# BGU-CS-VIL/DPMMSubClusters.jl

Hardware: AMD Instinct MI355X
Metric: Gibbs iterations/sec, N=10M D=64 NIW (higher is better)
Workload: dtype f32

## Files before the change

### dpmmsubclusters.jl_amd/csrc/dpmm_api.cpp

```cpp
#include "../../include/dpmm_hip.h"
#include "../../include/dpmm_hip_master.h"
#include "../../include/dpmm_hip_debug.h"
#include "../../include/dpmm_hip_tensor.h"
#include "../../include/dpmm_hip_csc.h"
#include "../../include/dpmm_hip_score.h"

#include <hip/hip_runtime.h>
#include <dlfcn.h>

#include <algorithm>
#include <atomic>
#include <condition_variable>
#include <mutex>
#include <thread>
#include <chrono>
#include <cmath>
#include <cstdio>
#include <cstring>
#include <cstdlib>
#include <ctime>
#include <string>
#include <unordered_map>
#include <vector>

// ... 1830 lines not shown
    }
    if (armed && wd_disarm(c)) {
        c->err = "collective timed out: a peer rank is gone or stuck (communicator aborted after DPMM_OPT_COMM_TIMEOUT_MS)";
        return DPMM_ECOMM;
    }
    if (c->comm_aborted.load(std::memory_order_relaxed) && rc == DPMM_OK && master_records_marked(sm, nrec)) return fail(c, DPMM_ECOMM, "communicator aborted");
    return rc;
}

int dpmm_debug_set_prelaunch_hook(void (*fn)(void *), void *arg) {
    dpmm::g_prelaunch_arg = arg;
    dpmm::g_prelaunch = fn;
    return DPMM_OK;
}

int dpmm_debug_counters(dpmm_ctx *c, int64_t *out, int n) {
    if (!c || !out || n < 1) return DPMM_EINVAL;
    for (int i = 0; i < n; ++i) out[i] = 0;
    out[0] = c->dbg_early_wait;
    return DPMM_OK;
}

int dpmm_step_master_device(dpmm_ctx *c, uint32_t reset_epoch, const int32_t *slots, uint32_t draw_epoch, const uint8_t **bad, const double **small) {
    if (!c || !slots || !bad || !small) return DPMM_EINVAL;
    if (!c->master) return fail(c, DPMM_ESTATE, "dpmm_niw_master_setup first");
    const int K = c->K;
    if (K < 1) return fail(c, DPMM_ESTATE, "no clusters");
    HIPCHK(c, hipSetDevice(c->device));
    int top = 0;
    for (int k = 0; k < K; ++k) {
        if (slots[k] < 0 || slots[k] >= DPMM_MAX_CLUSTERS) return fail(c, DPMM_EINVAL, "slot out of range");
        top = std::max(top, slots[k] + 1);
    }
    if (int rc = noise_flush(c)) return rc;
    if (int rc = master_capacity(c, top, draw_epoch ? K : 0)) return rc;
    if (int rc = spec_join(c)) return rc;
    c->spec_valid = false;
    const size_t out_bytes = sizeof(double) * 2 * (size_t)K * (size_t)c->packed_stride;
    if (int rc = ensure_out(c, DPMM_MAX_CLUSTERS + 64)) return rc;
    const size_t jobs_bytes = (sizeof(int32_t) * 2 * (size_t)K + 63) & ~(size_t)63;
    if (int rc = master_pinned(c, jobs_bytes + sizeof(double) * 3 * DPMM_MASTER_NSCALARS * (size_t)K)) return rc;
    std::vector<int32_t> jobs(2 * (size_t)K);
    for (int k = 0; k < K; ++k) { jobs[2 * k] = k; jobs[2 * k + 1] = slots[k]; }
    if (int rc = device_list(c, c->d_jobs, c->jobs_shadow, jobs.data(), jobs.size())) return rc;
    if (draw_epoch) if (int rc = device_list(c, c->d_dslots, c->dslots_shadow, slots, (size_t)K)) return rc;
    for (int32_t sl : c->apairs_req) if (sl >= top) { c->apairs_req.clear(); break; }
    const int napairs = (int)(c->apairs_req.size() / 2);
    c->apairs_valid = false;
    bool fuse_pairs = true;
    if (napairs > 0) {
        if ((size_t)napairs > c->apairs_cap) {
            HIPCHK(c, sync_stream(c, c->stream));
            HIPCHK(c, hipStreamSynchronize(c->stream2));
            size_t cap = 64;
            while (cap < (size_t)napairs) cap *= 2;
            hipFree(c->d_apairs); c->d_apairs = nullptr;
            if (c->h_apairs) hipHostFree(c->h_apairs);
            c->h_apairs = nullptr; c->apairs_cap = 0; c->apairs_shadow.clear();
            HIPCHK(c, hipMalloc(&c->d_apairs, sizeof(int32_t) * 2 * cap));
            HIPCHK(c, hipHostMalloc((void **)&c->h_apairs, sizeof(double) * DPMM_MASTER_NSCALARS * cap, hipHostMallocDefault));
            c->apairs_cap = cap;
        }
        if (c->ma.DP > 128 && (size_t)napairs > c->pair_cap) {
            HIPCHK(c, sync_stream(c, c->stream));
            HIPCHK(c, hipStreamSynchronize(c->stream2));
            hipFree(c->d_pairs); c->d_pairs = nullptr; c->pair_cap = 0;
            size_t cap = 64;
            while (cap < (size_t)napairs) cap *= 2;
            HIPCHK(c, hipMalloc(&c->d_pairs, sizeof(double) * cap * (size_t)c->ma.DP * (size_t)c->ma.DP));
            c->pair_cap = cap;
        }
        if (niw_master_can_fuse_pairs(c->ma)) {
            std::vector<int32_t> inv((size_t)top, -1), kp(c->apairs_req.size());
            for (int k = 0; k < K; ++k) inv[slots[k]] = k;
            for (size_t i = 0; i < kp.size(); ++i) {
                kp[i] = inv[c->apairs_req[i]];
                if (kp[i] < 0) { fuse_pairs = false; break; }
            }
            if (fuse_pairs) {
                if (c->opt_chain & 4) {
                    if (!(c->apairs_shadow.size() == kp.size() && memcmp(c->apairs_shadow.data(), kp.data(), sizeof(int32_t) * kp.size()) == 0) || !c->apairs_pinned_cur) {
                        c->apairs_shadow.assign(kp.begin(), kp.end());
                        c->apairs_pin_flip ^= 1;
                        int32_t *&buf = c->h_apairs_list[c->apairs_pin_flip];
                        size_t &cap = c->h_apairs_list_cap[c->apairs_pin_flip];
                        if (kp.size() > cap) {
                            if (buf) HIPCHK(c, hipHostFree(buf));
                            buf = nullptr; cap = 0;
                            size_t nc = 2048;
                            while (nc < kp.size()) nc *= 2;
                            HIPCHK(c, hipHostMalloc((void **)&buf, sizeof(int32_t) * nc, hipHostMallocDefault));
                            cap = nc;
                        }
                        memcpy(buf, kp.data(), sizeof(int32_t) * kp.size());
                        c->apairs_pinned_cur = buf;
                    }
                } else {
                    if (c->apairs_pinned_cur) { c->apairs_shadow.clear(); c->apairs_pinned_cur = nullptr; }
                    if (int rc = device_list(c, c->d_apairs, c->apairs_shadow, kp.data(), kp.size())) return rc;
                }
            }
        } else fuse_pairs = false;
        if (!fuse_pairs) {
            if (c->apairs_pinned_cur) { c->apairs_shadow.clear(); c->apairs_pinned_cur = nullptr; }
            if (int rc = device_list(c, c->d_apairs, c->apairs_shadow, c->apairs_req.data(), c->apairs_req.size(), c->stream2)) return rc;
        }
    } else fuse_pairs = false;
    double *sm = reinterpret_cast<double *>(c->h_master + jobs_bytes);
    master_mark_records(sm, 3 * (int64_t)K);
    const bool poll = c->opt_master_poll != 0;
    bool flags_sent = false;
    if (int rc = run_stats(c, nullptr, 0, true, reset_epoch, reinterpret_cast<uint8_t *>(c->h_out), &flags_sent)) return rc;
    if (!flags_sent) HIPCHK(c, launch_copy_bytes(c->h_out, reinterpret_cast<const uint8_t *>(c->d_out) + out_bytes, (size_t)K + 1, c->stream));
    const bool noise_in_post = draw_epoch != 0 && (c->opt_chain & 16) != 0 && niw_master_can_fuse_pairs(c->ma);
    bool normals_by_post = false;
    if (noise_in_post) {
        if (int rc = noise_join(c)) return rc;
        c->noise_valid = false;
    }
    if ((napairs > 0 && fuse_pairs) || noise_in_post) {
        const int nfp = fuse_pairs ? napairs : 0;
        if (poll && nfp > 0) master_mark_records(c->h_apairs, nfp);
        HIPCHK(c, launch_niw_master_posterior_pairs(c->ma, c->d_jobs, K, c->d_out, sm, ((c->opt_chain & 4) && c->apairs_pinned_cur) ? c->apairs_pinned_cur : c->d_apairs, nfp, c->h_apairs, c->stream,
                                                    noise_in_post ? 3 * K : 0, draw_epoch, noise_in_post ? c->d_Y[c->draw_cur ^ 1] : nullptr));
        normals_by_post = noise_in_post;
    } else HIPCHK(c, launch_niw_master_posterior(c->ma, c->d_jobs, K, c->d_out, sm, c->stream));
    if (napairs > 0 && fuse_pairs) {
        c->apairs_index.clear();
        for (int p = 0; p < napairs; ++p) c->apairs_index[((uint32_t)c->apairs_req[2 * p] << 16) | (uint32_t)c->apairs_req[2 * p + 1]] = p;
        c->apairs_dirty.assign((size_t)c->master_slots, 0);
        c->apairs_inflight = false; c->apairs_valid = true;
        c->apairs_req.clear();
    }
    const bool fused_pairs_launched = napairs > 0 && fuse_pairs;
    const bool need_event = !poll || (napairs > 0 && !fuse_pairs);
    if (need_event) HIPCHK(c, hipEventRecord(c->ev_master, c->stream));
    if (napairs > 0 && !fuse_pairs) {
        HIPCHK(c, hipStreamWaitEvent(c->stream2, c->ev_master, 0));
        HIPCHK(c, launch_niw_master_pairs(c->ma, c->d_apairs, napairs, c->d_pairs, c->h_apairs, c->stream2));
        HIPCHK(c, hipEventRecord(c->ev_pairs, c->stream2));
        c->apairs_index.clear();
        for (int p = 0; p < napairs; ++p) c->apairs_index[((uint32_t)c->apairs_req[2 * p] << 16) | (uint32_t)c->apairs_req[2 * p + 1]] = p;
        c->apairs_dirty.assign((size_t)c->master_slots, 0);
        c->apairs_inflight = true; c->apairs_valid = true;
        c->apairs_req.clear();
    }
    if (draw_epoch) {
        const int32_t *hs = c->d_dslots;
        const bool have_normals = normals_by_post || noise_ready(c, draw_epoch, K, c->draw_cur ^ 1);
        if (int rc = noise_join(c)) return rc;
        NiwMasterArgs ma = c->ma;
        ma.mu_draw = c->d_mu_draw[c->draw_cur ^ 1];
        HIPCHK(c, launch_niw_master_draw(ma, hs, K, draw_epoch, c->d_Y[c->draw_cur ^ 1], c->d_ld_sigma[c->draw_cur ^ 1], nullptr, nullptr,
                                         nullptr, nullptr, nullptr, nullptr, c->NB, nullptr, 1 | (have_normals ? 4 : 0), c->stream));
        c->noise_valid = false;
        c->spec_inflight = false; c->spec_valid = true; c->spec_epoch = draw_epoch;
        c->spec_slots.assign(slots, slots + K);
    }
    if (int rc = flush_undo(c)) return rc;
    if (poll) { if (int rc = wait_master_records(c, sm, 3 * (int64_t)K, c->h_apairs, fused_pairs_launched ? napairs : 0)) return rc; }
    else HIPCHK(c, sync_event(c, c->ev_master));
    if (master_marks_left(sm, K)) {
        ++c->dbg_early_wait;
        const auto t0 = std::chrono::steady_clock::now();
        while (master_marks_left(sm, K)) {
            if (std::chrono::steady_clock::now() - t0 > std::chrono::seconds(5)) return fail(c, DPMM_EHIP, "posterior records missing 5 s after the event wait returned");
            HIPCHK(c, sync_stream(c, c->stream));
        }
    }
    c->handover_inflight = false;
    *bad = reinterpret_cast<const uint8_t *>(c->h_out);
    *small = sm;
    return DPMM_OK;
}

int dpmm_suffstats_device(dpmm_ctx *c, const int64_t *idx, int n_idx) {
    if (!c) return DPMM_EINVAL;
    if (!c->master) return fail(c, DPMM_ESTATE, "dpmm_niw_master_setup first");
    return run_stats(c, idx, n_idx);
}

int dpmm_niw_master_posterior(dpmm_ctx *c, const int64_t *clusters, const int32_t *slots, int n, const double **small) {
    if (!c || !slots || !small || n < 0) return DPMM_EINVAL;
    if (!c->master) return fail(c, DPMM_ESTATE, "dpmm_niw_master_setup first");
    if (n == 0) { *small = nullptr; return DPMM_OK; }
    HIPCHK(c, hipSetDevice(c->device));
    int top = 0;
    for (int i = 0; i < n; ++i) {
        const int64_t k = clusters ? clusters[i] : i + 1;
        if (k < 1 || k > c->K) return fail(c, DPMM_EINVAL, "cluster index out of range");
        if (slots[i] < 0 || slots[i] >= DPMM_MAX_CLUSTERS) return fail(c, DPMM_EINVAL, "slot out of range");
        top = std::max(top, slots[i] + 1);
    }
    if (int rc = master_capacity(c, top, 0)) return rc;
    if (int rc = spec_join(c)) return rc;
    c->spec_valid = false;
    for (int i = 0; i < n; ++i) if ((size_t)slots[i] < c->apairs_dirty.size()) c->apairs_dirty[slots[i]] = 1;
    const size_t jobs_bytes = (sizeof(int32_t) * 2 * (size_t)n + 63) & ~(size_t)63;
    if (int rc = master_pinned(c, jobs_bytes + sizeof(double) * 3 * DPMM_MASTER_NSCALARS * (size_t)n)) return rc;
    HIPCHK(c, sync_stream(c, c->stream));
    std::vector<int32_t> jobs(2 * (size_t)n);
    for (int i = 0; i < n; ++i) { jobs[2 * i] = (int32_t)((clusters ? clusters[i] : i + 1) - 1); jobs[2 * i + 1] = slots[i]; }
    if (int rc = device_list(c, c->d_jobs, c->jobs_shadow, jobs.data(), jobs.size())) return rc;
    double *sm = reinterpret_cast<double *>(c->h_master + jobs_bytes);
    HIPCHK(c, launch_niw_master_posterior(c->ma, c->d_jobs, n, c->d_out, sm, c->stream));
    HIPCHK(c, sync_stream(c, c->stream));
    *small = sm;
    return DPMM_OK;
}

int dpmm_niw_master_draw(dpmm_ctx *c, uint32_t epoch, int K, const int32_t *slot_of_cluster, const float *lr, const float *w) {
    if (!c || !slot_of_cluster || !lr || !w) return DPMM_EINVAL;
    if (!c->master) return fail(c, DPMM_ESTATE, "dpmm_niw_master_setup first");
    if (int rc = check_K(c, K)) return rc;
    HIPCHK(c, hipSetDevice(c->device));
    for (int k = 0; k < K; ++k)
        if (slot_of_cluster[k] < 0 || slot_of_cluster[k] >= c->master_slots) return fail(c, DPMM_EINVAL, "slot without a posterior on the device");
    if (int rc = noise_flush(c)) return rc;
    if (int rc = ensure_capacity(c, K)) return rc;
    if (int rc = master_capacity(c, 0, K)) return rc;
    if (c->handover_inflight) HIPCHK(c, sync_stream(c, c->stream));
    c->handover_inflight = true;
    float *hlr = reinterpret_cast<float *>(c->h_draw), *hw = hlr + 2 * K;
    memcpy(hlr, lr, sizeof(float) * 2 * K);
    memcpy(hw, w, sizeof(float) * K);
    c->have_tail = c->opt_tail && c->D >= 4 && c->D % 4 == 0 && K > 1;
    const bool ahead = c->spec_valid && c->spec_epoch == epoch && (int)c->spec_slots.size() == K &&
                       memcmp(c->spec_slots.data(), slot_of_cluster, sizeof(int32_t) * K) == 0;
    if (int rc = spec_join(c)) return rc;
    c->spec_valid = false;
    if (int rc = noise_join(c)) return rc;
    if (!ahead) if (int rc = device_list(c, c->d_dslots, c->dslots_shadow, slot_of_cluster, (size_t)K)) return rc;
    const int32_t *hs = c->d_dslots;
    c->draw_cur ^= 1;
    NiwMasterArgs ma = c->ma;
    ma.mu_draw = c->d_mu_draw[c->draw_cur];
    const bool normals = !ahead && noise_ready(c, epoch, K, c->draw_cur);
    c->predictive = false;
    const bool roles = (c->opt_chain & 2) != 0, b3_in_pack = roles && want_b3_images(c), pb_in_pack = b3_in_pack && want_pair_ball(c, K);
    HIPCHK(c, launch_niw_master_draw(ma, hs, K, epoch, c->d_Y[c->draw_cur], c->d_ld_sigma[c->draw_cur], hlr, hw, c->d_Rp, c->d_mup, c->d_cst,
                                     c->have_tail ? c->d_tail : nullptr, c->NB, c->d_work, (ahead ? 2 : (normals ? 7 : 3)) | (roles ? 8 : 0) | (b3_in_pack ? 16 : 0) | (pb_in_pack ? 32 : 0), c->stream));
    if (int rc = direction_tables(c, K, b3_in_pack, pb_in_pack)) return rc;
    c->noise_pending = c->opt_noise_ahead < 0 ? (c->D >= 128 || c->n < 4000000) : c->opt_noise_ahead != 0; c->noise_pend_epoch = epoch + 1; c->noise_pend_nmat = 3 * std::min(K + 4, c->master_K);
    if ((c->opt_chain & 16) && niw_master_can_fuse_pairs(c->ma)) c->noise_pending = false;
    c->work_zeroed = true;
    c->have_screen_prep = false;
    c->K = K;
    c->have_params = true;
    c->predictive = false;
    c->draws_on_device = true;
    return DPMM_OK;
}

int dpmm_niw_master_pairs_ahead(dpmm_ctx *c, const int32_t *slots_i, const int32_t *slots_j, int n) {
    if (!c || n < 0 || (n > 0 && (!slots_i || !slots_j))) return DPMM_EINVAL;
    if (!c->master) return fail(c, DPMM_ESTATE, "dpmm_niw_master_setup first");
    c->apairs_req.clear();
    for (int i = 0; i < n; ++i) {
        if (slots_i[i] < 0 || slots_i[i] >= DPMM_MAX_CLUSTERS || slots_j[i] < 0 || slots_j[i] >= DPMM_MAX_CLUSTERS) { c->apairs_req.clear(); return fail(c, DPMM_EINVAL, "slot out of range"); }
        c->apairs_req.push_back(slots_i[i]); c->apairs_req.push_back(slots_j[i]);
    }
    return DPMM_OK;
}

int dpmm_niw_master_pairs(dpmm_ctx *c, const int32_t *slots_i, const int32_t *slots_j, int n, const double **small) {
    if (!c || !slots_i || !slots_j || !small || n < 0) return DPMM_EINVAL;
    if (!c->master) return fail(c, DPMM_ESTATE, "dpmm_niw_master_setup first");
    if (n == 0) { *small = nullptr; return DPMM_OK; }
    HIPCHK(c, hipSetDevice(c->device));
    for (int i = 0; i < n; ++i)
        if (slots_i[i] < 0 || slots_i[i] >= c->master_slots || slots_j[i] < 0 || slots_j[i] >= c->master_slots) return fail(c, DPMM_EINVAL, "slot out of range");
    const size_t DP = (size_t)c->ma.DP;
    if (c->apairs_valid) {
        bool all = true;
        std::vector<int> rec((size_t)n);
        for (int i = 0; i < n && all; ++i) {
            const auto it = c->apairs_index.find(((uint32_t)slots_i[i] << 16) | (uint32_t)slots_j[i]);
            all = it != c->apairs_index.end() && !c->apairs_dirty[slots_i[i]] && !c->apairs_dirty[slots_j[i]];
            if (all) rec[i] = it->second;
        }
        if (all) {
            if (int rc = master_pinned(c, sizeof(double) * DPMM_MASTER_NSCALARS * (size_t)n)) return rc;
            HIPCHK(c, hipEventSynchronize(c->ev_pairs));
            double *sm = reinterpret_cast<double *>(c->h_master);
            for (int i = 0; i < n; ++i) memcpy(sm + (size_t)i * DPMM_MASTER_NSCALARS, c->h_apairs + (size_t)rec[i] * DPMM_MASTER_NSCALARS, sizeof(double) * DPMM_MASTER_NSCALARS);
            *small = sm;
            return DPMM_OK;
        }
    }
    if (int rc = spec_join(c)) return rc;
    if ((size_t)n > c->pair_cap) {
        HIPCHK(c, sync_stream(c, c->stream));
        HIPCHK(c, hipStreamSynchronize(c->stream2));
        hipFree(c->d_pairs); c->d_pairs = nullptr; c->pair_cap = 0;
        size_t cap = 64;
        while (cap < (size_t)n) cap *= 2;
        HIPCHK(c, hipMalloc(&c->d_pairs, sizeof(double) * cap * DP * DP));
        c->pair_cap = cap;
    }
    const size_t idx_bytes = (sizeof(int32_t) * 2 * (size_t)n + 63) & ~(size_t)63;
    if (int rc = master_pinned(c, idx_bytes + sizeof(double) * DPMM_MASTER_NSCALARS * (size_t)n)) return rc;
    HIPCHK(c, sync_stream(c, c->stream));
    int32_t *pr = reinterpret_cast<int32_t *>(c->h_master);
    for (int i = 0; i < n; ++i) { pr[2 * i] = slots_i[i]; pr[2 * i + 1] = slots_j[i]; }
    double *sm = reinterpret_cast<double *>(c->h_master + idx_bytes);
    HIPCHK(c, launch_niw_master_pairs(c->ma, pr, n, c->d_pairs, sm, c->stream));
    HIPCHK(c, sync_stream(c, c->stream));
    *small = sm;
    return DPMM_OK;
}

int dpmm_niw_master_put_rows(dpmm_ctx *c, const double *rows, int K) {
    if (!c || !rows) return DPMM_EINVAL;
    if (!c->master) return fail(c, DPMM_ESTATE, "dpmm_niw_master_setup first");
    if (int rc = check_K(c, K)) return rc;
    HIPCHK(c, hipSetDevice(c->device));
    if (int rc = ensure_capacity(c, K)) return rc;
    HIPCHK(c, sync_stream(c, c->stream));
    HIPCHK(c, hipMemcpy(c->d_out, rows, sizeof(double) * 2 * (size_t)K * (size_t)c->packed_stride, hipMemcpyHostToDevice));
    c->apairs_valid = false;
    if (K != c->K) c->have_params = false;
    c->K = K;
    return DPMM_OK;
}

int dpmm_niw_master_rows(dpmm_ctx *c, const int32_t *slots, int n, double *out) {
    if (!c || !slots || !out || n < 0) return DPMM_EINVAL;
    if (!c->master) return fail(c, DPMM_ESTATE, "dpmm_niw_master_setup first");
    if (n == 0) return DPMM_OK;
    HIPCHK(c, hipSetDevice(c->device));
    const size_t stride = (size_t)c->packed_stride, bytes = sizeof(double) * 2 * (size_t)n * stride;
    for (int i = 0; i < n; ++i)
        if (slots[i] < 0 || slots[i] >= c->master_slots) return fail(c, DPMM_EINVAL, "slot out of range");
    if (int rc = ensure_out(c, bytes)) return rc;
    if (int rc = ensure_pinned(c, sizeof(int32_t) * (size_t)n + 64)) return rc;
    HIPCHK(c, sync_stream(c, c->stream));
    memcpy(c->h_pin, slots, sizeof(int32_t) * (size_t)n);
    HIPCHK(c, launch_niw_rows_gather(c->ma.rows_store, reinterpret_cast<const int32_t *>(c->h_pin), n, (int64_t)stride,
                                     reinterpret_cast<double *>(c->h_out), c->stream));
    HIPCHK(c, sync_stream(c, c->stream));
    memcpy(out, c->h_out, bytes);
    return DPMM_OK;
}

int dpmm_niw_master_draws(dpmm_ctx *c, int K, float *mu, float *R, float *logdet) {
    if (!c || !mu || !R || !logdet) return DPMM_EINVAL;
    if (!c->master || !c->draws_on_device || K != c->K) return fail(c, DPMM_ESTATE, "no device draws for this K");
    HIPCHK(c, hipSetDevice(c->device));
    HIPCHK(c, sync_stream(c, c->stream));
    const size_t D = (size_t)c->D, DP = (size_t)c->ma.DP;
    std::vector<double> Y(3 * (size_t)K * DP * DP);
    std::vector<float> m(3 * (size_t)K * DP);
    HIPCHK(c, hipMemcpy(Y.data(), c->d_Y[c->draw_cur], sizeof(double) * Y.size(), hipMemcpyDeviceToHost));
    HIPCHK(c, hipMemcpy(m.data(), c->d_mu_draw[c->draw_cur], sizeof(float) * m.size(), hipMemcpyDeviceToHost));
    HIPCHK(c, hipMemcpy(logdet, c->d_ld_sigma[c->draw_cur], sizeof(float) * 3 * (size_t)K, hipMemcpyDeviceToHost));
    for (size_t j = 0; j < 3 * (size_t)K; ++j) {
        for (size_t d = 0; d < D; ++d) mu[j * D + d] = m[j * DP + d];
        for (size_t r = 0; r < D; ++r)
            for (size_t cc = 0; cc < D; ++cc) R[(j * D + r) * D + cc] = cc >= r ? (float)Y[(j * DP + cc) * DP + r] : 0.f;
    }
    return DPMM_OK;
}

int dpmm_mult_master_setup(dpmm_ctx *c, const float *alpha, const float *alpha_outlier) {
    if (!c || !alpha) return DPMM_EINVAL;
    if (c->prior != DPMM_PRIOR_MULT) return fail(c, DPMM_EINVAL, "dpmm_mult_master_setup: the context is not Multinomial");
    if (c->D > DPMM_MULT_MASTER_MAXD) return fail(c, DPMM_ELIMIT, "D exceeds the device Dirichlet draw's limit");
    HIPCHK(c, hipSetDevice(c->device));
    HIPCHK(c, sync_stream(c, c->stream));
    if (!c->d_malpha) HIPCHK(c, hipMalloc(&c->d_malpha, sizeof(float) * 2 * (size_t)c->ldx));
    HIPCHK(c, hipMemsetAsync(c->d_malpha, 0, sizeof(float) * 2 * (size_t)c->ldx, c->stream));
    HIPCHK(c, sync_stream(c, c->stream));
    HIPCHK(c, hipMemcpy(c->d_malpha, alpha, sizeof(float) * (size_t)c->D, hipMemcpyHostToDevice));
    if (alpha_outlier) HIPCHK(c, hipMemcpy(c->d_malpha + c->ldx, alpha_outlier, sizeof(float) * (size_t)c->D, hipMemcpyHostToDevice));
    c->mult_has_alpha1 = alpha_outlier != nullptr;
    for (int p = 0; p < 2; ++p) {
        const float *al = p ? alpha_outlier : alpha;
        double sa = 0.0, sl = 0.0;
        if (al) for (int d = 0; d < c->D; ++d) { sa += (double)al[d]; sl += lgamma((double)al[d]); }
        c->mult_prior_c[2 * p] = sa; c->mult_prior_c[2 * p + 1] = sl;
    }
    if (!c->d_mpairs) HIPCHK(c, hipMalloc(&c->d_mpairs, sizeof(int32_t) * 2 * DPMM_MULT_MASTER_MAXPAIRS));
    if (!c->h_marg) HIPCHK(c, hipHostMalloc((void **)&c->h_marg, sizeof(double) * (6 * DPMM_MAX_CLUSTERS + DPMM_MULT_MASTER_MAXPAIRS), hipHostMallocDefault));
    c->marg_valid = false; c->marg_req = false; c->mpairs_shadow.clear();
    if (!c->h_draw) HIPCHK(c, hipHostMalloc((void **)&c->h_draw, sizeof(float) * 3 * DPMM_MAX_CLUSTERS, hipHostMallocDefault));
    c->mult_master = true;
    return DPMM_OK;
}

int dpmm_mult_master_put_rows(dpmm_ctx *c, const double *rows, int K) {
    if (!c || !rows) return DPMM_EINVAL;
    if (!c->mult_master) return fail(c, DPMM_ESTATE, "dpmm_mult_master_setup first");
    if (int rc = check_K(c, K)) return rc;
    HIPCHK(c, hipSetDevice(c->device));
// ... 1063 lines not shown
```

### dpmmsubclusters.jl_amd/csrc/niw_master.hip

```cpp
#include <algorithm>
#include "dpmm_device.h"
#include "dpmm_kernels.h"
#include "niw_b3.h"

namespace dpmm {

enum : uint32_t { STREAM_M_NORMAL = 32, STREAM_M_CHI = 33, STREAM_M_XI = 34 };
typedef double f64x4m __attribute__((ext_vector_type(4)));
constexpr int NS = DPMM_MASTER_NSCALARS;

__device__ __forceinline__ double log_mv_gamma_wave(double x, int D, int lane) {
    double t = 0.0;
    for (int d = 1 + lane; d <= D; d += 64) t += lgamma(x + 0.5 * (double)(1 - d));
    for (int o = 32; o > 0; o >>= 1) t += __shfl_xor(t, o);
    return t + (double)D * (double)(D - 1) * 0.25 * 1.1447298858494001741434273513530587;
}

__device__ __forceinline__ double u53(uint32_t a, uint32_t b) {
    return ((double)((((uint64_t)a << 32) | b) >> 11) + 0.5) * (1.0 / 9007199254740992.0);
}
__device__ __forceinline__ double normal_from(const Philox4 &r) {
    const double u1 = u53(r.v[0], r.v[1]), u2 = u53(r.v[2], r.v[3]);
    return sqrt(-2.0 * log(u1)) * cos(6.283185307179586476925 * u2);
}
// ... 319 lines not shown
    double *Lp = xi + DP;
    if (!have_noise) {
        const int HP = DP / 2;
        for (int p2 = tid; p2 < DP * HP; p2 += 256) {
            const int r = p2 / HP, c = 2 * (p2 - r * HP);
            double n0, n1;
            bartlett_pair(A, id, epoch, r, c, n0, n1);
            Y[(int64_t)r * DP + c] = n0; Y[(int64_t)r * DP + c + 1] = n1;
        }
    }
    __syncthreads();
    for (int r = tid; r < D; r += 256) Y[(int64_t)r * DP + r] = bartlett_diag(A.seed, id, epoch, r, nu);
    for (int d = tid; d < DP; d += 256)
        xi[d] = d < D ? normal_from(philox4x32_10(A.seed, (id << 32) + (uint64_t)d, epoch, STREAM_M_XI)) : 0.0;
    __syncthreads();
    DSTAMP(Dn = __builtin_amdgcn_s_memtime() - D0;)
    { const int a2 = tid >> 4, b2 = tid & 15; const double dv = L[(int64_t)a2 * DP + b2]; Ld[a2 * 17 + b2] = (b2 <= a2) ? dv : 0.0; if (a2 == b2) Ld[a2 * 17 + 16] = 1.0 / dv; }
    __syncthreads();
    for (int ib = 0; ib < NB; ++ib) {
        const int i0 = 16 * ib, ncol = i0 + 16;
        DSTAMP(Da = __builtin_amdgcn_s_memtime();)
        DSTAMP(Db = __builtin_amdgcn_s_memtime(); Ds += Db - Da;)
        {
            const int wave = tid >> 6, li = tid & 15, lg = (tid >> 4) & 3;
            for (int idx = 0; idx <= ib; ++idx) {
                const int turn = idx & 7;
                if ((turn < 4 ? turn : 7 - turn) != wave) continue;
                const int cb = idx;
                const double *yc = Y + (int64_t)lg * DP + 16 * cb + li;
                f64x4m acc = {yc[(int64_t)(i0 + 0) * DP], yc[(int64_t)(i0 + 4) * DP], yc[(int64_t)(i0 + 8) * DP], yc[(int64_t)(i0 + 12) * DP]};
                const double *lp = Lp + lg * 17 + li;
                constexpr int PG = 5;
                const int nch = ib - cb;
                double bA[PG][4], bB[PG][4];
                auto loadg = [&](double (&buf)[PG][4], int ch0) {
#pragma unroll
                    for (int g2 = 0; g2 < PG; ++g2) {
                        const int ch = ch0 + g2 < nch ? ch0 + g2 : nch - 1;
#pragma unroll
                        for (int u = 0; u < 4; ++u) buf[g2][u] = yc[(int64_t)(16 * (cb + ch) + 4 * u) * DP];
                    }
                };
                auto mm = [&](const double (&buf)[PG][4], int ch0) {
#pragma unroll
                    for (int g2 = 0; g2 < PG; ++g2)
                        if (ch0 + g2 < nch) {
#pragma unroll
                            for (int u = 0; u < 4; ++u)
                                acc = __builtin_amdgcn_mfma_f64_16x16x4f64(-lp[(16 * (cb + ch0 + g2) + 4 * u) * 17], buf[g2][u], acc, 0, 0, 0);
                        }
                };
                if (nch > 0) {
                    loadg(bA, 0);
                    for (int ch0 = 0; ch0 < nch; ch0 += 2 * PG) {
                        if (ch0 + PG < nch) loadg(bB, ch0 + PG);
                        mm(bA, ch0);
                        if (ch0 + 2 * PG < nch) loadg(bA, ch0 + 2 * PG);
                        if (ch0 + PG < nch) mm(bB, ch0 + PG);
                    }
                }
                double *tp = T + lg * DP + 16 * cb + li;
                tp[0] = acc[0]; tp[4 * DP] = acc[1]; tp[8 * DP] = acc[2]; tp[12 * DP] = acc[3];
            }
        }
        __syncthreads();
        DSTAMP(Da = __builtin_amdgcn_s_memtime(); Dp += Da - Db;)
        const int n0 = i0 + 16;
        const bool more = ib + 1 < NB;
        double lnx[16], dnx = 0.0;
        {
            const int kc = (more && tid < n0) ? tid : 0, rb = more ? n0 : 0;
#pragma unroll
            for (int a2 = 0; a2 < 16; ++a2) lnx[a2] = L[(int64_t)(rb + a2) * DP + kc];
            dnx = L[(int64_t)(rb + (tid >> 4)) * DP + rb + (tid & 15)];
        }
        for (int q = tid; q < ncol; q += 256) {
            double t[16];
#pragma unroll
            for (int r = 0; r < 16; ++r) t[r] = T[r * DP + q];
#pragma unroll
            for (int r = 0; r < 16; ++r) {
                const double yv = t[r] * Ld[r * 17 + 16];
                t[r] = yv;
#pragma unroll
                for (int r2 = r + 1; r2 < 16; ++r2) t[r2] = __builtin_fma(-Ld[r2 * 17 + r], yv, t[r2]);
            }
#pragma unroll
            for (int r = 0; r < 16; ++r) Y[(int64_t)(i0 + r) * DP + q] = (q <= i0 + r) ? t[r] : 0.0;
        }
        __syncthreads();
        if (more) {
            if (tid < n0) {
#pragma unroll
                for (int a2 = 0; a2 < 16; ++a2) Lp[tid * 17 + a2] = lnx[a2];
            }
            const int a2 = tid >> 4, b2 = tid & 15;
            Ld[a2 * 17 + b2] = (b2 <= a2) ? dnx : 0.0;
            if (a2 == b2) Ld[a2 * 17 + 16] = 1.0 / dnx;
        }
        __syncthreads();
        DSTAMP(Dt += __builtin_amdgcn_s_memtime() - Da;)
    }
    DSTAMP(Da = __builtin_amdgcn_s_memtime();)
    if (tid < 64) {
        double lg = 0.0;
        for (int d = tid; d < D; d += 64) lg += log(Y[(int64_t)d * DP + d]);
        for (int o = 32; o > 0; o >>= 1) lg += __shfl_xor(lg, o);
        if (tid == 0) logdet_sigma[blockIdx.x] = (float)(-2.0 * lg);
    }
    double *vv = T;
    __syncthreads();
    for (int cb = NB - 1; cb >= 0; --cb) {
        const int c0 = 16 * cb;
        { const int a2 = tid >> 4, b2 = tid & 15; Ld[a2 * 17 + b2] = (b2 <= a2) ? Y[(int64_t)(c0 + a2) * DP + c0 + b2] : 0.0; }
        double yr[16];
        const int rr = tid < c0 ? tid : 0;
#pragma unroll
        for (int a2 = 0; a2 < 16; ++a2) yr[a2] = Y[(int64_t)(c0 + a2) * DP + rr];
        __syncthreads();
        if (tid < 64) {
            const int t16 = tid & 15;
            double xb = xi[c0 + t16];
            const double inv = 1.0 / Ld[t16 * 17 + t16];
            double col[16];
#pragma unroll
            for (int a2 = 0; a2 < 16; ++a2) col[a2] = a2 > t16 ? Ld[a2 * 17 + t16] : 0.0;
            double mine_v = 0.0;
#pragma unroll
            for (int a2 = 15; a2 >= 0; --a2) {
                const double wq = xb * inv;
                const double va = __hiloint2double(__builtin_amdgcn_readlane(__double2hiint(wq), a2), __builtin_amdgcn_readlane(__double2loint(wq), a2));
                mine_v = t16 == a2 ? va : mine_v;
                xb = __builtin_fma(-va, col[a2], xb);
            }
            if (tid < 16) vv[c0 + tid] = mine_v;
        }
        __syncthreads();
        for (int r = tid; r < c0; r += 256) {
            double acc = xi[r];
#pragma unroll
            for (int a2 = 0; a2 < 16; ++a2) acc = __builtin_fma(-vv[c0 + a2], yr[a2], acc);
            xi[r] = acc;
        }
        __syncthreads();
    }
    const double isk = 1.0 / sqrt(kap);
    const double *m = A.mean + (int64_t)row * DP;
    float *mu_out = A.mu_draw + (int64_t)blockIdx.x * DP;
    for (int d = tid; d < DP; d += 256) mu_out[d] = d < D ? (float)(m[d] + vv[d] * isk) : 0.f;
#ifdef DPMM_POST_STAMPS
    __syncthreads();
    if (tid == 0 && blockIdx.x == 3) { float *o = logdet_sigma + 3; o[0] = (float)Dn; o[1] = (float)Ds; o[2] = (float)Dp; o[3] = (float)Dt; o[4] = (float)(__builtin_amdgcn_s_memtime() - Da); o[5] = (float)(__builtin_amdgcn_s_memtime() - D0); }
#endif
}

__global__ __launch_bounds__(256) void niw_draw_inputs_kernel(NiwMasterArgs A, const int32_t *__restrict__ slot_of_cluster, uint32_t epoch,
                                                              double *__restrict__ Aout, double *__restrict__ xiout) {
    const int k = blockIdx.x / 3, w = blockIdx.x % 3;
    const int row = 3 * slot_of_cluster[k] + w;
    const int D = A.D, DP = A.DP, HP = DP / 2, tid = threadIdx.x;
    const double nu = A.nu[row];
    const uint64_t id = (uint64_t)blockIdx.x;
    double *Ao = Aout + (int64_t)blockIdx.x * D * D;
    for (int p2 = tid; p2 < DP * HP; p2 += 256) {
        const int r = p2 / HP, c = 2 * (p2 - r * HP);
        double n0, n1;
        bartlett_pair(A, id, epoch, r, c, n0, n1);
        if (r < D && c < D && c != r) Ao[(int64_t)r * D + c] = n0;
        if (r < D && c + 1 < D && c + 1 != r) Ao[(int64_t)r * D + c + 1] = n1;
    }
    for (int r = tid; r < D; r += 256) Ao[(int64_t)r * D + r] = bartlett_diag(A.seed, id, epoch, r, nu);
    for (int d = tid; d < D; d += 256)
        xiout[(int64_t)blockIdx.x * D + d] = normal_from(philox4x32_10(A.seed, (id << 32) + (uint64_t)d, epoch, STREAM_M_XI));
}
hipError_t launch_niw_draw_inputs(const NiwMasterArgs &a, const int32_t *slot_of_cluster, int K, uint32_t epoch, double *Aout, double *xiout, hipStream_t s) {
    DPMM_LAUNCH(niw_draw_inputs_kernel, dim3(3 * K), dim3(256), 0, s, a, slot_of_cluster, epoch, Aout, xiout);
    return hipGetLastError();
}

__global__ void niw_master_pack_kernel(const double *__restrict__ Yall, const float *__restrict__ mu_draw, const float *__restrict__ logdet_sigma,
                                       const float *__restrict__ lr, const float *__restrict__ wts, float *__restrict__ Rp,
                                       float *__restrict__ mup, float *__restrict__ cst, float *__restrict__ tail, int D, int DPm, int NB,
                                       int nmat, unsigned long long *__restrict__ work) {
    const int NP = NB * (NB + 1) / 2;
    const int DP = 16 * NB;
    if (work && blockIdx.x == 0 && threadIdx.x < 8) { work[threadIdx.x] = 0ull; work[8 + 16 * threadIdx.x] = 0ull; }
    for (int64_t e = blockIdx.x * (int64_t)blockDim.x + threadIdx.x; e < nmat; e += (int64_t)gridDim.x * blockDim.x) {
        const int k = (int)(e / 3), w = (int)(e % 3);
        const float lw = w == 0 ? logf(wts[k]) : logf(lr[2 * k + (w - 1)]);
        cst[e] = -0.5f * logdet_sigma[e] + lw;
    }
    const int64_t total = (int64_t)nmat * NP * 256;
    for (int64_t e = blockIdx.x * (int64_t)blockDim.x + threadIdx.x; e < total; e += (int64_t)gridDim.x * blockDim.x) {
        const int jj = (int)(e & 3);
        const int lane = (int)((e >> 2) & 63);
        const int64_t pj = e >> 8;
        const int pair = (int)(pj % NP);
        const int j = (int)(pj / NP);
        int bi = 0, rem = pair;
        while (rem >= NB - bi) { rem -= NB - bi; ++bi; }
        const int t = bi + rem;
        const int row = 16 * bi + (lane & 15);
        const int col = 16 * t + 4 * (lane >> 4) + jj;
        float v = 0.f;
        if (row < D && col < D && col >= row) v = (float)Yall[(int64_t)j * DPm * DPm + (int64_t)col * DPm + row];
        Rp[e] = v;
    }
    const int64_t totmu = (int64_t)nmat * DP;
    for (int64_t e = blockIdx.x * (int64_t)blockDim.x + threadIdx.x; e < totmu; e += (int64_t)gridDim.x * blockDim.x) {
        const int d = (int)(e % DP);
        const int64_t j = e / DP;
        mup[e] = d < D ? mu_draw[j * DPm + d] : 0.f;
    }
    if (tail && D >= 4) {
        const int f0 = D - 4, K = nmat / 3, NPR = (K + 1) / 2;
        for (int64_t e = blockIdx.x * (int64_t)blockDim.x + threadIdx.x; e < (int64_t)NPR * 32; e += (int64_t)gridDim.x * blockDim.x) {
            const int c = (int)(e & 1), q = (int)((e >> 1) & 15), k = 2 * (int)(e >> 5) + c;
            const int64_t j = k < K ? 3 * k : 0;
            const int tr[10] = {0, 0, 0, 0, 1, 1, 1, 2, 2, 3}, tc[10] = {0, 1, 2, 3, 1, 2, 3, 2, 3, 3};
            float v = 0.f;
            if (k >= K) v = (q == 14) ? -INFINITY : 0.f;
            else if (q < 10) v = (float)Yall[j * DPm * DPm + (int64_t)(f0 + tc[q]) * DPm + (f0 + tr[q])];
            else if (q < 14) v = mu_draw[j * DPm + f0 + (q - 10)];
            else if (q == 14) {
                v = -0.5f * logdet_sigma[j] + logf(wts[k]);
            }
            tail[e] = v;
        }
        float *ball = tail + 32 * NPR;
        for (int64_t e = blockIdx.x * (int64_t)blockDim.x + threadIdx.x; e < (int64_t)K * 16; e += (int64_t)gridDim.x * blockDim.x) {
            const int q = (int)(e & 15), k = (int)(e >> 4);
            const int64_t j = 3 * (int64_t)k;
            const int tr[10] = {0, 0, 0, 0, 1, 1, 1, 2, 2, 3}, tc[10] = {0, 1, 2, 3, 1, 2, 3, 2, 3, 3};
            float v;
            if (q < 4) v = mu_draw[j * DPm + f0 + q];
            else if (q < 14) v = (float)Yall[j * DPm * DPm + (int64_t)(f0 + tc[q - 4]) * DPm + (f0 + tr[q - 4])];
            else if (q == 14) {
                float t10[10];
                for (int i = 0; i < 10; ++i) t10[i] = (float)Yall[j * DPm * DPm + (int64_t)(f0 + tc[i]) * DPm + (f0 + tr[i])];
                v = tail_opnorm_bound(t10);
            } else v = -0.5f * logdet_sigma[j] + logf(wts[k]);
            ball[e] = v;
        }
        if (NB == 4) {
            uint32_t *refb = reinterpret_cast<uint32_t *>(ball + 16 * (size_t)K);
            for (int64_t e = blockIdx.x * (int64_t)blockDim.x + threadIdx.x; e < (int64_t)K * REFB_WORDS; e += (int64_t)gridDim.x * blockDim.x) {
                const int64_t j = 3 * (e / REFB_WORDS);
                int row, c0, c1;
                refb_map((int)(e % REFB_WORDS), row, c0, c1);
                const float v0 = (row < D && c0 < D && c0 >= row) ? (float)Yall[j * DPm * DPm + (int64_t)c0 * DPm + row] : 0.f;
                const float v1 = (row < D && c1 < D && c1 >= row) ? (float)Yall[j * DPm * DPm + (int64_t)c1 * DPm + row] : 0.f;
                refb[e] = bf16_rne_bits(v0) | (bf16_rne_bits(v1) << 16);
            }
        }
    }
}

struct PackRoles { int first[7]; };
__global__ __launch_bounds__(256) void niw_master_pack_roles_kernel(const double *__restrict__ Yall, const float *__restrict__ mu_draw, const float *__restrict__ logdet_sigma,
                                                                    const float *__restrict__ lr, const float *__restrict__ wts, float *__restrict__ Rp,
                                                                    float *__restrict__ mup, float *__restrict__ cst, float *__restrict__ tail, int D, int DPm, int NB,
                                                                    int nmat, unsigned long long *__restrict__ work, PackRoles R, int with_b3) {
    const int NP = NB * (NB + 1) / 2;
    const int DP = 16 * NB;
    const int K = nmat / 3;
    int role = 0;
    while (role < 5 && (int)blockIdx.x >= R.first[role + 1]) ++role;
    const int64_t t0 = ((int64_t)blockIdx.x - R.first[role]) * 256 + threadIdx.x, stride = (int64_t)(R.first[role + 1] - R.first[role]) * 256;
    auto Rel = [&](int64_t j, int row, int col) -> float {
        return (row < D && col < D && col >= row) ? (float)Yall[j * DPm * DPm + (int64_t)col * DPm + row] : 0.f;
    };
    if (role == 0) {
        const int64_t total4 = (int64_t)nmat * NP * 64;
        for (int64_t u = t0; u < total4; u += stride) {
            const int lane = (int)(u & 63);
            const int64_t pj = u >> 6;
            const int pair = (int)(pj % NP);
            const int64_t j = pj / NP;
            int bi = 0, rem = pair;
            while (rem >= NB - bi) { rem -= NB - bi; ++bi; }
            const int t = bi + rem;
            const int row = 16 * bi + (lane & 15), col = 16 * t + 4 * (lane >> 4);
            float4 v;
            v.x = Rel(j, row, col); v.y = Rel(j, row, col + 1); v.z = Rel(j, row, col + 2); v.w = Rel(j, row, col + 3);
            reinterpret_cast<float4 *>(Rp)[u] = v;
        }
        return;
    }
    if (role == 1) {
        if (work && t0 < 8) { work[t0] = 0ull; work[8 + 16 * t0] = 0ull; }
        const bool tl = tail && D >= 4;
        const int f0 = D - 4, NPR = (K + 1) / 2;
        const int64_t n0 = nmat, n1 = n0 + (int64_t)nmat * DP, n2 = n1 + (tl ? (int64_t)NPR * 32 : 0), n3 = n2 + (tl ? (int64_t)K * 16 : 0);
        const int tr[10] = {0, 0, 0, 0, 1, 1, 1, 2, 2, 3}, tc[10] = {0, 1, 2, 3, 1, 2, 3, 2, 3, 3};
        for (int64_t i = t0; i < n3; i += stride) {
            if (i < n0) {
                const int k = (int)(i / 3), w = (int)(i % 3);
                const float lw = w == 0 ? logf(wts[k]) : logf(lr[2 * k + (w - 1)]);
                cst[i] = -0.5f * logdet_sigma[i] + lw;
            } else if (i < n1) {
                const int64_t e = i - n0;
                const int d = (int)(e % DP);
                const int64_t j = e / DP;
                mup[e] = d < D ? mu_draw[j * DPm + d] : 0.f;
            } else if (i < n2) {
                const int64_t e = i - n1;
// ... 298 lines not shown
                    const double wj = quad_bcast(wv[jj >> 2] * dv[jj], jj & 3);
                    if (sq == (jj & 3)) wv[jj >> 2] = wj;
#pragma unroll
                    for (int i2 = 0; i2 < 4; ++i2) {
                        if (4 * i2 + 3 < jj) wv[i2] = __builtin_fma(-cf[jj][i2], wj, wv[i2]);
                        else if (4 * i2 < jj) wv[i2] = (4 * i2 + sq < jj) ? __builtin_fma(-cf[jj][i2], wj, wv[i2]) : wv[i2];
                    }
                }
                if (q < j0) {
#pragma unroll
                    for (int i2 = 0; i2 < 4; ++i2) Pm[(j0 + 4 * i2 + sq) * LD + q] = wv[i2];
                }
            }
        }
        __syncthreads();
        PSTAMP(Ta = __builtin_amdgcn_s_memtime(); Tp += Ta - Tb;)
        {
            const int wave = tid >> 6, li = tid & 15, lg = (tid >> 4) & 3;
            for (int t = wave; t < jb * (jb + 1) / 2; t += 4) {
                int kb = 0;
                while ((kb + 1) * (kb + 2) / 2 <= t) ++kb;
                const int qb = t - kb * (kb + 1) / 2;
                double *cp = Pm + (16 * kb + lg) * LD + 16 * qb + li;
                f64x4m acc = {cp[0], cp[4 * LD], cp[8 * LD], cp[12 * LD]};
                const double *wa = Pm + (j0 + lg) * LD + 16 * kb + li, *wb = Pm + (j0 + lg) * LD + 16 * qb + li;
#pragma unroll
                for (int t4 = 0; t4 < 4; ++t4) acc = __builtin_amdgcn_mfma_f64_16x16x4f64(-wa[4 * t4 * LD], wb[4 * t4 * LD], acc, 0, 0, 0);
                cp[0] = acc[0]; cp[4 * LD] = acc[1]; cp[8 * LD] = acc[2]; cp[12 * LD] = acc[3];
            }
        }
        __syncthreads();
        PSTAMP(Tt += __builtin_amdgcn_s_memtime() - Ta;)
    }
    PSTAMP(Ta = __builtin_amdgcn_s_memtime();)
    if (tid < 64) {
        double lg = 0.0;
        for (int a = tid; a < DP; a += 64) lg += log(piv[a]);
        for (int o = 32; o > 0; o >>= 1) lg += __shfl_xor(lg, o);
        if (tid == 0) small[(int64_t)bid * NS + 3] = s_bad ? NAN : lg;
    } else if (tid < 128) {
        const double lm = log_mv_gamma_wave(0.5 * ((N == 0.0) ? v0 : v1), D, tid - 64);
        if (tid == 64) small[(int64_t)bid * NS + 4] = lm;
    }
    if constexpr (!PAIRS) {
        double *F = A.fac + (int64_t)row * DP * DP;
        for (int e = tid; e < DP * DP; e += 256) {
            const int a = e / DP, b = e - a * DP;
            F[e] = b <= a ? Pm[a * LD + b] : 0.0;
        }
    }
#ifdef DPMM_POST_STAMPS
    __syncthreads();
    if (tid == 0 && bid == 5) { double *o = small + 5 * NS; o[0] = (double)Tf; o[1] = (double)Td; o[2] = (double)Tp; o[3] = (double)Tt; }
    if (tid == 0 && bid == 6) { double *o = small + 6 * NS; o[0] = (double)(__builtin_amdgcn_s_memtime() - Ta); o[1] = (double)(__builtin_amdgcn_s_memtime() - T0); }
#endif
}
template <bool PAIRS>
__global__ __launch_bounds__(256) void niw_post_lds_kernel(NiwMasterArgs A, const int32_t *__restrict__ jobs, const double *__restrict__ rows,
                                                           double *__restrict__ small) {
    niw_post_lds_body<PAIRS>(A, jobs, rows, small, (int)blockIdx.x);
}
__global__ __launch_bounds__(256) void niw_post_both_kernel(NiwMasterArgs A, const int32_t *__restrict__ jobs, const double *__restrict__ rows,
                                                            double *__restrict__ small, int nposts, const int32_t *__restrict__ pair_jobs,
                                                            double *__restrict__ pair_small, int npairs, uint32_t noise_epoch, double *__restrict__ noise_Y, int nsplit) {
    if ((int)blockIdx.x < nposts) niw_post_lds_body<false>(A, jobs, rows, small, (int)blockIdx.x);
    else if ((int)blockIdx.x < nposts + npairs) niw_post_lds_body<true>(A, pair_jobs, rows, pair_small, (int)blockIdx.x - nposts);
    else {
        const int nb = (int)blockIdx.x - nposts - npairs, mat = nb / nsplit, part = nb - mat * nsplit;
        const int DP = A.DP, HP = DP / 2;
        double *Y = noise_Y + (int64_t)mat * DP * DP;
        for (int p2 = part * 256 + threadIdx.x; p2 < DP * HP; p2 += nsplit * 256) {
            const int r = p2 / HP, c = 2 * (p2 - r * HP);
            double n0, n1;
            bartlett_pair(A, (uint64_t)mat, noise_epoch, r, c, n0, n1);
            Y[(int64_t)r * DP + c] = n0; Y[(int64_t)r * DP + c + 1] = n1;
        }
    }
}
size_t niw_post_lds_bytes(int DP) { return sizeof(double) * ((size_t)DP * (DP + 1) + 3 * (size_t)DP + 16); }
constexpr int NIW_POST_LDS_MAXDP = 128;

bool niw_master_can_fuse_pairs(const NiwMasterArgs &a) { return a.DP <= NIW_POST_LDS_MAXDP; }
hipError_t launch_niw_master_posterior_pairs(const NiwMasterArgs &a, const int32_t *jobs, int njobs, const double *rows, double *small,
                                             const int32_t *cluster_pairs, int npairs, double *pair_small, hipStream_t s,
                                             int noise_nmat, uint32_t noise_epoch, double *noise_Y) {
    static bool attr = false;
    if (!attr) { hipFuncSetAttribute((const void *)niw_post_both_kernel, hipFuncAttributeMaxDynamicSharedMemorySize, (int)niw_post_lds_bytes(NIW_POST_LDS_MAXDP)); attr = true; }
    const int nsplit = a.DP >= 128 ? 8 : (a.DP >= 48 ? 4 : 1);
    const int nnoise = (noise_Y && noise_nmat > 0) ? noise_nmat * nsplit : 0;
    DPMM_LAUNCH(niw_post_both_kernel, dim3(3 * njobs + npairs + nnoise), dim3(256), niw_post_lds_bytes(a.DP), s, a, jobs, rows, small, 3 * njobs,
                       cluster_pairs, pair_small, npairs, noise_epoch, noise_Y, nsplit);
    return hipGetLastError();
}
hipError_t launch_niw_master_pairs(const NiwMasterArgs &a, const int32_t *pairs, int n, double *scratch, double *small, hipStream_t s) {
    if (n <= 0) return hipSuccess;
    if (a.DP <= NIW_POST_LDS_MAXDP) {
        static bool attr = false;
        if (!attr) { hipFuncSetAttribute((const void *)niw_post_lds_kernel<true>, hipFuncAttributeMaxDynamicSharedMemorySize, (int)niw_post_lds_bytes(NIW_POST_LDS_MAXDP)); attr = true; }
        DPMM_LAUNCH(niw_post_lds_kernel<true>, dim3(n), dim3(256), niw_post_lds_bytes(a.DP), s, a, pairs, (const double *)nullptr, small);
        return hipGetLastError();
    }
    DPMM_LAUNCH(niw_form_pair_kernel, dim3(n, a.DP >= 64 ? 16 : 1), dim3(256), 0, s, a, pairs, scratch, small);
    NiwMasterArgs b = a;
    b.fac = scratch;
    DPMM_LAUNCH(niw_chol_kernel, dim3(n), dim3(256), niw_master_lds_bytes(a.DP), s, b, (const int32_t *)nullptr, small);
    return hipGetLastError();
}

__global__ void niw_rows_gather_kernel(const double *__restrict__ rows_store, const int32_t *__restrict__ slots, int n, int64_t two_stride,
                                       double *__restrict__ dst) {
    const int64_t total = (int64_t)n * two_stride;
    for (int64_t e = blockIdx.x * (int64_t)blockDim.x + threadIdx.x; e < total; e += (int64_t)gridDim.x * blockDim.x) {
        const int i = (int)(e / two_stride);
        dst[e] = rows_store[(int64_t)slots[i] * two_stride + (e - (int64_t)i * two_stride)];
    }
}
hipError_t launch_niw_rows_gather(const double *rows_store, const int32_t *slots, int n, int64_t stride, double *dst, hipStream_t s) {
    const int64_t total = (int64_t)n * 2 * stride;
    const int grid = (int)std::min<int64_t>(4096, (total + 255) / 256);
    DPMM_LAUNCH(niw_rows_gather_kernel, dim3(grid > 0 ? grid : 1), dim3(256), 0, s, rows_store, slots, n, 2 * stride, dst);
    return hipGetLastError();
}

size_t niw_master_lds_bytes(int DP) { return sizeof(double) * ((size_t)34 * DP + 16 * 17 + 256); }

hipError_t launch_niw_master_posterior(const NiwMasterArgs &a, const int32_t *jobs, int njobs, const double *rows, double *small, hipStream_t s) {
    if (njobs <= 0) return hipSuccess;
    if (a.DP <= NIW_POST_LDS_MAXDP) {
        static bool attr_l = false;
        if (!attr_l) { hipFuncSetAttribute((const void *)niw_post_lds_kernel<false>, hipFuncAttributeMaxDynamicSharedMemorySize, (int)niw_post_lds_bytes(NIW_POST_LDS_MAXDP)); attr_l = true; }
        DPMM_LAUNCH(niw_post_lds_kernel<false>, dim3(3 * njobs), dim3(256), niw_post_lds_bytes(a.DP), s, a, jobs, rows, small);
        return hipGetLastError();
    }
    DPMM_LAUNCH(niw_form_kernel, dim3(3 * njobs, a.DP >= 64 ? 16 : 1), dim3(256), 0, s, a, jobs, rows, small);
    static bool attr = false;
    if (!attr) {
        hipFuncSetAttribute((const void *)niw_chol_kernel, hipFuncAttributeMaxDynamicSharedMemorySize, (int)niw_master_lds_bytes(DPMM_MASTER_MAXD));
        hipFuncSetAttribute((const void *)niw_draw_kernel, hipFuncAttributeMaxDynamicSharedMemorySize, (int)niw_master_lds_bytes(DPMM_MASTER_MAXD));
        attr = true;
    }
    DPMM_LAUNCH(niw_chol_kernel, dim3(3 * njobs), dim3(256), niw_master_lds_bytes(a.DP), s, a, jobs, small);
    return hipGetLastError();
}

hipError_t launch_niw_master_draw(const NiwMasterArgs &a, const int32_t *slot_of_cluster, int K, uint32_t epoch, double *Y, float *logdet_sigma,
                                  const float *lr, const float *wts, float *Rp, float *mup, float *cst, float *tail, int NB,
                                  unsigned long long *work, int what, hipStream_t s) {
    static bool attr = false;
    if (!attr) {
        hipFuncSetAttribute((const void *)niw_chol_kernel, hipFuncAttributeMaxDynamicSharedMemorySize, (int)niw_master_lds_bytes(DPMM_MASTER_MAXD));
        hipFuncSetAttribute((const void *)niw_draw_kernel, hipFuncAttributeMaxDynamicSharedMemorySize, (int)niw_master_lds_bytes(DPMM_MASTER_MAXD));
        attr = true;
    }
    if (what & 1) DPMM_LAUNCH(niw_draw_kernel, dim3(3 * K), dim3(256), niw_master_lds_bytes(a.DP), s, a, slot_of_cluster, epoch, Y, logdet_sigma, (what & 4) ? 1 : 0);
    if ((what & 2) && (what & 8)) {
        const int nmat = 3 * K, NP = NB * (NB + 1) / 2, DPs = 16 * NB;
        const bool tl = tail != nullptr && a.D >= 4;
        auto blocks = [](int64_t items, int cap) -> int { return (int)std::max<int64_t>(1, std::min<int64_t>((items + 255) / 256, cap)); };
        PackRoles R;
        R.first[0] = 0;
        R.first[1] = R.first[0] + blocks((int64_t)nmat * NP * 64, 2048);
        R.first[2] = R.first[1] + blocks((int64_t)nmat * (1 + DPs) + (tl ? (int64_t)((K + 1) / 2) * 32 + (int64_t)K * 16 : 0), 512);
        const bool img = tl && NB == 4;
        R.first[3] = R.first[2] + (img ? blocks((int64_t)K * REFB_WORDS, 1024) : 0);
        const bool b3 = img && (what & 16);
        R.first[4] = R.first[3] + (b3 ? blocks((int64_t)2 * K * REFB_WORDS, 2048) : 0);
        R.first[5] = R.first[4] + (b3 ? blocks((int64_t)2 * K * 256, 256) : 0);
        const bool pb = b3 && (what & 32) && K >= 2 && K <= PB_MAXK;
        R.first[6] = R.first[5] + (pb ? K : 0);
        DPMM_LAUNCH(niw_master_pack_roles_kernel, dim3(R.first[6]), dim3(256), 0, s, Y, a.mu_draw, logdet_sigma, lr, wts, Rp, mup, cst, tail, a.D, a.DP, NB,
                    nmat, work, R, b3 ? 1 : 0);
    } else if (what & 2) DPMM_LAUNCH(niw_master_pack_kernel, dim3(512), dim3(256), 0, s, Y, a.mu_draw, logdet_sigma, lr, wts, Rp, mup, cst, tail, a.D, a.DP, NB,
                                     3 * K, work);
    return hipGetLastError();
}

}
```

Before: 697.8.

## Add LDS-resident MFMA triangular-solve draw kernel behind opt_chain flag

Adds an alternative NIW posterior draw kernel for DP<=64 that stages the Cholesky factor and Bartlett matrix in padded LDS and runs a blocked triangular solve with f64 MFMA plus a wave-level back-substitution, using one wave per block by default. It is enabled only when opt_chain bit 64 is set; otherwise the existing 256-thread draw kernel runs. The aim is to cut global-memory traffic and synchronisation in the per-cluster draw, at the cost of less parallelism per block and extra LDS use.

```diff
diff --git a/dpmmsubclusters.jl_amd/csrc/dpmm_api.cpp b/dpmmsubclusters.jl_amd/csrc/dpmm_api.cpp
--- a/dpmmsubclusters.jl_amd/csrc/dpmm_api.cpp
+++ b/dpmmsubclusters.jl_amd/csrc/dpmm_api.cpp
@@ -2006,7 +2006,7 @@
         NiwMasterArgs ma = c->ma;
         ma.mu_draw = c->d_mu_draw[c->draw_cur ^ 1];
         HIPCHK(c, launch_niw_master_draw(ma, hs, K, draw_epoch, c->d_Y[c->draw_cur ^ 1], c->d_ld_sigma[c->draw_cur ^ 1], nullptr, nullptr,
-                                         nullptr, nullptr, nullptr, nullptr, c->NB, nullptr, 1 | (have_normals ? 4 : 0), c->stream));
+                                         nullptr, nullptr, nullptr, nullptr, c->NB, nullptr, 1 | (have_normals ? 4 : 0) | ((c->opt_chain & 64) ? 64 : 0), c->stream));
         c->noise_valid = false;
         c->spec_inflight = false; c->spec_valid = true; c->spec_epoch = draw_epoch;
         c->spec_slots.assign(slots, slots + K);
@@ -2093,7 +2093,7 @@
     c->predictive = false;
     const bool roles = (c->opt_chain & 2) != 0, b3_in_pack = roles && want_b3_images(c), pb_in_pack = b3_in_pack && want_pair_ball(c, K);
     HIPCHK(c, launch_niw_master_draw(ma, hs, K, epoch, c->d_Y[c->draw_cur], c->d_ld_sigma[c->draw_cur], hlr, hw, c->d_Rp, c->d_mup, c->d_cst,
-                                     c->have_tail ? c->d_tail : nullptr, c->NB, c->d_work, (ahead ? 2 : (normals ? 7 : 3)) | (roles ? 8 : 0) | (b3_in_pack ? 16 : 0) | (pb_in_pack ? 32 : 0), c->stream));
+                                     c->have_tail ? c->d_tail : nullptr, c->NB, c->d_work, (ahead ? 2 : (normals ? 7 : 3)) | (roles ? 8 : 0) | (b3_in_pack ? 16 : 0) | (pb_in_pack ? 32 : 0) | ((c->opt_chain & 64) ? 64 : 0), c->stream));
     if (int rc = direction_tables(c, K, b3_in_pack, pb_in_pack)) return rc;
     c->noise_pending = c->opt_noise_ahead < 0 ? (c->D >= 128 || c->n < 4000000) : c->opt_noise_ahead != 0; c->noise_pend_epoch = epoch + 1; c->noise_pend_nmat = 3 * std::min(K + 4, c->master_K);
     if ((c->opt_chain & 16) && niw_master_can_fuse_pairs(c->ma)) c->noise_pending = false;
diff --git a/dpmmsubclusters.jl_amd/csrc/niw_master.hip b/dpmmsubclusters.jl_amd/csrc/niw_master.hip
--- a/dpmmsubclusters.jl_amd/csrc/niw_master.hip
+++ b/dpmmsubclusters.jl_amd/csrc/niw_master.hip
@@ -495,6 +495,135 @@
     __syncthreads();
     if (tid == 0 && blockIdx.x == 3) { float *o = logdet_sigma + 3; o[0] = (float)Dn; o[1] = (float)Ds; o[2] = (float)Dp; o[3] = (float)Dt; o[4] = (float)(__builtin_amdgcn_s_memtime() - Da); o[5] = (float)(__builtin_amdgcn_s_memtime() - D0); }
 #endif
+}
+
+constexpr int NIW_DRAW_LDS_MAXDP = 64;
+#ifndef DPMM_DRAW_WAVES
+#define DPMM_DRAW_WAVES 1
+#endif
+size_t niw_draw_lds_bytes(int DP) { return sizeof(double) * (2 * (size_t)DP * (DP + 1) + 16 * (size_t)DP + 3 * (size_t)DP); }
+template <int NT>
+__global__ __launch_bounds__(NT) void niw_draw_lds_kernel(NiwMasterArgs A, const int32_t *__restrict__ slot_of_cluster, uint32_t epoch,
+                                                          double *__restrict__ Yall, float *__restrict__ logdet_sigma, int have_noise) {
+    constexpr int NW = NT / 64;
+    const int k = blockIdx.x / 3, w = blockIdx.x % 3;
+    const int row = 3 * slot_of_cluster[k] + w;
+    const int D = A.D, DP = A.DP, NB = DP / 16, LD = DP + 1, tid = threadIdx.x;
+    const double *Lg = A.fac + (int64_t)row * DP * DP;
+    double *Yg = Yall + (int64_t)blockIdx.x * DP * DP;
+    const double nu = A.nu[row], kap = A.kap[row];
+    const uint64_t id = (uint64_t)blockIdx.x;
+    extern __shared__ double lds[];
+    double *Ls = lds;
+    double *Ys = Ls + (size_t)DP * LD;
+    double *T = Ys + (size_t)DP * LD;
+    double *xi = T + 16 * DP;
+    double *vv = xi + DP;
+    double *dinv = vv + DP;
+    const int rr = tid >> 6, cc = tid & 63;
+    for (int a0 = rr; a0 < DP; a0 += 16 * NW) {
+        double lv[16], yv[16];
+#pragma unroll
+        for (int u = 0; u < 16; ++u) {
+            const int a = a0 + u * NW;
+            const bool on = a < DP && cc < DP;
+            lv[u] = on ? Lg[(int64_t)a * DP + cc] : 0.0;
+            yv[u] = (on && have_noise) ? Yg[(int64_t)a * DP + cc] : 0.0;
+        }
+#pragma unroll
+        for (int u = 0; u < 16; ++u) {
+            const int a = a0 + u * NW;
+            if (a < DP && cc < DP) { Ls[a * LD + cc] = lv[u]; Ys[a * LD + cc] = yv[u]; }
+        }
+    }
+    if (!have_noise) {
+        __syncthreads();
+        const int HP = DP / 2;
+        for (int p2 = tid; p2 < DP * HP; p2 += NT) {
+            const int r = p2 / HP, c = 2 * (p2 - r * HP);
+            double n0, n1;
+            bartlett_pair(A, id, epoch, r, c, n0, n1);
+            Ys[r * LD + c] = n0; Ys[r * LD + c + 1] = n1;
+        }
+    }
+    __syncthreads();
+    for (int r = tid; r < D; r += NT) Ys[r * LD + r] = bartlett_diag(A.seed, id, epoch, r, nu);
+    for (int d = tid; d < DP; d += NT) {
+        xi[d] = d < D ? normal_from(philox4x32_10(A.seed, (id << 32) + (uint64_t)d, epoch, STREAM_M_XI)) : 0.0;
+        dinv[d] = 1.0 / Ls[d * LD + d];
+    }
+    __syncthreads();
+    const int wave = __builtin_amdgcn_readfirstlane(tid >> 6), li = tid & 15, lg = (tid >> 4) & 3;
+    for (int ib = 0; ib < NB; ++ib) {
+        const int i0 = 16 * ib, ncol = i0 + 16;
+        for (int cb = wave; cb <= ib; cb += NW) {
+            const double *yc = Ys + lg * LD + 16 * cb + li;
+            f64x4m acc = {yc[(i0 + 0) * LD], yc[(i0 + 4) * LD], yc[(i0 + 8) * LD], yc[(i0 + 12) * LD]};
+            const double *lp = Ls + (i0 + li) * LD + lg;
+            for (int kk = 16 * cb; kk < i0; kk += 16) {
+#pragma unroll
+                for (int u = 0; u < 4; ++u) acc = __builtin_amdgcn_mfma_f64_16x16x4f64(-lp[kk + 4 * u], yc[(kk + 4 * u) * LD], acc, 0, 0, 0);
+            }
+            double *tp = T + lg * DP + 16 * cb + li;
+            tp[0] = acc[0]; tp[4 * DP] = acc[1]; tp[8 * DP] = acc[2]; tp[12 * DP] = acc[3];
+        }
+        __syncthreads();
+        for (int q = tid; q < ncol; q += NT) {
+            double t[16];
+#pragma unroll
+            for (int r = 0; r < 16; ++r) t[r] = T[r * DP + q];
+#pragma unroll
+            for (int r = 0; r < 16; ++r) {
+                const double yv = t[r] * dinv[i0 + r];
+                t[r] = yv;
+#pragma unroll
+                for (int r2 = r + 1; r2 < 16; ++r2) t[r2] = __builtin_fma(-Ls[(i0 + r2) * LD + i0 + r], yv, t[r2]);
+            }
+#pragma unroll
+            for (int r = 0; r < 16; ++r) Ys[(i0 + r) * LD + q] = (q <= i0 + r) ? t[r] : 0.0;
+        }
+        __syncthreads();
+    }
+    if (tid < 64) {
+        double lgs = 0.0;
+        for (int d = tid; d < D; d += 64) lgs += log(Ys[d * LD + d]);
+        for (int o = 32; o > 0; o >>= 1) lgs += __shfl_xor(lgs, o);
+        if (tid == 0) logdet_sigma[blockIdx.x] = (float)(-2.0 * lgs);
+    }
+    for (int cb = NB - 1; cb >= 0; --cb) {
+        const int c0 = 16 * cb;
+        if (tid < 64) {
+            const int t16 = tid & 15;
+            double xb = xi[c0 + t16];
+            const double inv = 1.0 / Ys[(c0 + t16) * LD + c0 + t16];
+            double col[16];
+#pragma unroll
+            for (int a2 = 0; a2 < 16; ++a2) col[a2] = a2 > t16 ? Ys[(c0 + a2) * LD + c0 + t16] : 0.0;
+            double mine_v = 0.0;
+#pragma unroll
+            for (int a2 = 15; a2 >= 0; --a2) {
+                const double wq = xb * inv;
+                const double va = __hiloint2double(__builtin_amdgcn_readlane(__double2hiint(wq), a2), __builtin_amdgcn_readlane(__double2loint(wq), a2));
+                mine_v = t16 == a2 ? va : mine_v;
+                xb = __builtin_fma(-va, col[a2], xb);
+            }
+            if (tid < 16) vv[c0 + tid] = mine_v;
+        }
+        __syncthreads();
+        for (int r = tid; r < c0; r += NT) {
+            double acc = xi[r];
+#pragma unroll
+            for (int a2 = 0; a2 < 16; ++a2) acc = __builtin_fma(-vv[c0 + a2], Ys[(c0 + a2) * LD + r], acc);
+            xi[r] = acc;
+        }
+        __syncthreads();
+    }
+    const double isk = 1.0 / sqrt(kap);
+    const double *m = A.mean + (int64_t)row * DP;
+    float *mu_out = A.mu_draw + (int64_t)blockIdx.x * DP;
+    for (int d = tid; d < DP; d += NT) mu_out[d] = d < D ? (float)(m[d] + vv[d] * isk) : 0.f;
+    for (int a = rr; a < DP; a += NW)
+        if (cc < DP) Yg[(int64_t)a * DP + cc] = cc <= a ? Ys[a * LD + cc] : 0.0;
 }
 
 __global__ __launch_bounds__(256) void niw_draw_inputs_kernel(NiwMasterArgs A, const int32_t *__restrict__ slot_of_cluster, uint32_t epoch,
@@ -1099,7 +1228,12 @@
         hipFuncSetAttribute((const void *)niw_draw_kernel, hipFuncAttributeMaxDynamicSharedMemorySize, (int)niw_master_lds_bytes(DPMM_MASTER_MAXD));
         attr = true;
     }
-    if (what & 1) DPMM_LAUNCH(niw_draw_kernel, dim3(3 * K), dim3(256), niw_master_lds_bytes(a.DP), s, a, slot_of_cluster, epoch, Y, logdet_sigma, (what & 4) ? 1 : 0);
+    if ((what & 1) && (what & 64) && a.DP <= NIW_DRAW_LDS_MAXDP) {
+        constexpr int NT = 64 * DPMM_DRAW_WAVES;
+        static bool attr_w = false;
+        if (!attr_w) { hipFuncSetAttribute((const void *)niw_draw_lds_kernel<NT>, hipFuncAttributeMaxDynamicSharedMemorySize, (int)niw_draw_lds_bytes(NIW_DRAW_LDS_MAXDP)); attr_w = true; }
+        DPMM_LAUNCH(niw_draw_lds_kernel<NT>, dim3(3 * K), dim3(NT), niw_draw_lds_bytes(a.DP), s, a, slot_of_cluster, epoch, Y, logdet_sigma, (what & 4) ? 1 : 0);
+    } else if (what & 1) DPMM_LAUNCH(niw_draw_kernel, dim3(3 * K), dim3(256), niw_master_lds_bytes(a.DP), s, a, slot_of_cluster, epoch, Y, logdet_sigma, (what & 4) ? 1 : 0);
     if ((what & 2) && (what & 8)) {
         const int nmat = 3 * K, NP = NB * (NB + 1) / 2, DPs = 16 * NB;
         const bool tl = tail != nullptr && a.D >= 4;
```

Measured after the change: 690.6. 0.99x the previous value.
